# tangkk/audiomod

Hardware: NVIDIA B200
Metric: audio-sec/sec, 2048-pt PV pitch-shift, batched streams (higher is better)
Workload: dtype f32

## Files before the change

audiomod_b200/csrc/pv_engine.cu:

```cuda
#include <cuda_runtime.h>

#include <algorithm>
#include <chrono>
#include <cmath>
#include <cstdarg>
#include <cstdio>
#include <cstdlib>
#include <cstring>
#include <condition_variable>
#include <exception>
#include <functional>
#include <map>
#include <memory>
#include <mutex>
#include <new>
#include <string>
#include <thread>
#include <vector>

#include "../../include/pvgpu.h"
#include "pv_internal.h"
#include "pv_kernels.cuh"
#include "pv_plan.h"

#ifndef M_PI
#define M_PI 3.14159265358979323846
#endif

namespace pvgpu {

static thread_local std::string g_err;
const std::string &last_error_string() { return g_err; }
int fail(int code, const char *fmt, ...) {
    char buf[512];
    va_list ap;
    va_start(ap, fmt);
    vsnprintf(buf, sizeof buf, fmt, ap);
    va_end(ap);
    g_err = buf;
    return code;
}
template <class F> static int guarded(F f) {
    try {
        return f();
    } catch (const std::bad_alloc &) {
        return fail(PVGPU_ENOMEM, "out of host memory");
    } catch (const std::exception &e) {
        return fail(PVGPU_ESTATE, "unexpected failure: %s", e.what());
    }
}
#define CU(call)                                                                                      \
    do {                                                                                              \
        cudaError_t e_ = (call);                                                                      \
        if (e_ != cudaSuccess) return fail(e_ == cudaErrorMemoryAllocation ? PVGPU_ENOMEM : PVGPU_ECUDA, \
                                           "%s: %s (%s:%d)", #call, cudaGetErrorString(e_), __FILE__, __LINE__); \
    } while (0)

struct DevBuf {
    void *p = nullptr;
    size_t bytes = 0;
    ~DevBuf() { release(); }
    void release() { if (p) cudaFree(p); p = nullptr; bytes = 0; }
    cudaError_t ensure(size_t n) {
        if (n <= bytes) return cudaSuccess;
        release();
        cudaError_t e = cudaMalloc(&p, n);
        if (e == cudaSuccess) bytes = n;
        return e;
    }
    template <typename T> T *as() const { return (T *)p; }
};

struct PinnedArena {
    char *base = nullptr;
    size_t cap = 0, used = 0;
    ~PinnedArena() { if (base) cudaFreeHost(base); }
    void reserve(size_t bytes) {
        used = 0;
        if (bytes <= cap) return;
        if (base) cudaFreeHost(base);
        base = nullptr; cap = 0;
        const size_t want = bytes + bytes / 2 + 4096;
        if (cudaHostAlloc((void **)&base, want, cudaHostAllocDefault) == cudaSuccess) cap = want;
        else { cudaGetLastError(); base = nullptr; }
    }
    void *take(size_t bytes) {
        bytes = (bytes + 63) & ~(size_t)63;
        if (!base || used + bytes > cap) return nullptr;
        void *p = base + used;
        used += bytes;
        return p;
    }
};

static Config to_config(const pvgpu_config &c) {
    Config k;
    k.sample_rate = c.sample_rate; k.channels = c.channels; k.time_ratio = c.time_ratio; k.pitch_semitones = c.pitch_semitones;
    k.mode = c.mode; k.coremode = c.coremode; k.fftsize = c.fftsize; k.hopsize = c.hopsize;
    return k;
}

static int validate(const pvgpu_config *cfg) {
    if (!cfg) return fail(PVGPU_EINVAL, "null config");
    if (cfg->channels < 1 || cfg->channels > 16) return fail(PVGPU_EINVAL, "channels must be 1..16");
    if (cfg->sample_rate < 1000) return fail(PVGPU_EINVAL, "sample_rate too small");
    if (cfg->fftsize < 16 || cfg->fftsize > 16384) return fail(PVGPU_EINVAL, "fftsize must be 16..16384");
    return PVGPU_OK;
}

static void fill_info(const Derived &d, pvgpu_info *info) {
    info->fftsize = d.N; info->hop = d.hop; info->bins = d.H;
    info->pitch_scale = d.pitch_scale; info->hs_ratio = d.hs;
    info->resampler_active = d.rs.active ? 1 : 0;
    info->resampler_filt_len = (int)d.rs.filt_len;
    info->resampler_num = d.rs.num; info->resampler_den = d.rs.den;
    info->outbuf_capacity = d.outbuf_cap;
}

struct Pipeline {
    Derived d;
    Tables t;
    DevPlan p{};
    int device = 0;
    DevBuf b_window, b_twf, b_twi, b_stwf, b_stwi, b_perm, b_omega, b_rstab, b_rsquad, b_warp, b_tw2f, b_tw2i, b_tw3f, b_tw3i;
    DevBuf b_recs, b_norm, b_whisper, b_carmag, b_carph;
    long recs_base = 0, recs_count = 0;
    int64_t norm_base = 0;
    int max_consumed = 1;
    int max_out = 1;
    int ola_run = 16;
    bool fused = false;
    int fused_pref = -1;
    bool ola_ws = false;
    PostChain post{};
    FusedArgs fa{};
    std::vector<SliceRec> h_recs;
    DevBuf b_runs, b_rsent, b_rsfrac, b_rssteps;
    long run_origin = 0;
    int table_run = 1;
    int64_t launches = 0;
    bool profile = false;
    struct Span { int kind; cudaEvent_t a, b; };
    std::vector<Span> spans;
    size_t spans_used = 0;
    double kind_ms[8] = {0};
    int64_t kind_n[8] = {0};

    ~Pipeline() { for (auto &sp : spans) { cudaEventDestroy(sp.a); cudaEventDestroy(sp.b); } }

    Span *span_begin(int kind, cudaStream_t st) {
        if (!profile) return nullptr;
        if (spans_used == spans.size()) {
            Span sp{kind, nullptr, nullptr};
            if (cudaEventCreate(&sp.a) != cudaSuccess || cudaEventCreate(&sp.b) != cudaSuccess) return nullptr;
            spans.push_back(sp);
        }
        Span *sp = &spans[spans_used++];
        sp->kind = kind;
        cudaEventRecord(sp->a, st);
        return sp;
    }
    static void span_end(Span *sp, cudaStream_t st) { if (sp) cudaEventRecord(sp->b, st); }
    void collect_spans() {
        for (size_t i = 0; i < spans_used; ++i) {
            float ms = 0.f;
            if (cudaEventElapsedTime(&ms, spans[i].a, spans[i].b) == cudaSuccess) { kind_ms[spans[i].kind] += ms; kind_n[spans[i].kind] += 1; }
        }
        spans_used = 0;
    }

    int init(const pvgpu_config &cfg) {
        int ndev = 0;
        if (cudaGetDeviceCount(&ndev) != cudaSuccess || ndev == 0) return fail(PVGPU_ECUDA, "no CUDA device: the phase vocoder has no CPU fallback");
        if (cfg.device < 0 || cfg.device >= ndev) return fail(PVGPU_EINVAL, "device %d out of range (%d devices)", cfg.device, ndev);
        device = cfg.device;
        CU(cudaSetDevice(device));
        d = derive(to_config(cfg));
        if (d.hop < 1 || d.hop > d.N) return fail(PVGPU_EINVAL, "derived hop %d invalid for fft size %d", d.hop, d.N);
        t = make_tables(d.N, d.hop);
        if ((int)t.radix.size() > kMaxStages) return fail(PVGPU_EINVAL, "fft size too large");
        if (d.cepstral && !(d.N == 512 || d.N == 1024 || d.N == 2048 || d.N == 4096 || d.N == 8192))
            return fail(PVGPU_EINVAL, "the cepstral modes need an FFT size of 512..8192 (got %d)", d.N);
        CU(configure_kernels());
        p.N = d.N; p.H = d.H; p.half = d.N / 2; p.nc = d.N / 2; p.hop = d.hop;
        p.Hp = (d.H + 3) & ~3;
        p.nstages = (int)t.radix.size();
        for (int i = 0; i < p.nstages; ++i) { p.radix[i] = t.radix[i]; p.span[i] = t.span[i]; }
        p.inv_n = 1.f / d.N;
        p.two_pi_hop = 2 * M_PI * (size_t)d.hop;
        p.freq_comp = d.freq_comp;
        p.fixed_gain = d.fixed_gain;
        p.rs_active = (d.rs.active && !d.vocoder) ? 1 : 0;
        p.rs_direct = d.rs.direct ? 1 : 0;
        p.rs_num = d.rs.num; p.rs_den = d.rs.den; p.rs_filt_len = d.rs.filt_len; p.rs_oversample = d.rs.oversample;
        p.rs_int_adv = d.rs.int_adv; p.rs_frac_adv = d.rs.frac_adv;
        p.rs_table_len = (int)d.rs.table.size();
        if (!(d.robotic || d.whisper || d.vocoder || d.constant_mode) && d.cfg.coremode != 2 &&
            !(d.cfg.coremode == 1 && lock_smem_bytes(p, d.cfg.channels, max_peaks()) <= (size_t)200 * 1024) &&
            smem_phase_core(p, d.cfg.channels, max_peaks()) + 64 > (size_t)200 * 1024)
            return fail(PVGPU_EINVAL, "%d channels at FFT size %d need more shared memory per stream than the device has (the phase core keeps every channel's phase state on chip)",
                        d.cfg.channels, d.N);
        int rc;
        if ((rc = upload(b_window, t.window.data(), sizeof(float) * t.window.size()))) return rc;
        if ((rc = upload(b_twf, t.tw_fwd.data(), sizeof(float) * t.tw_fwd.size()))) return rc;
        if ((rc = upload(b_twi, t.tw_inv.data(), sizeof(float) * t.tw_inv.size()))) return rc;
        if ((rc = upload(b_stwf, t.stw_fwd.data(), sizeof(float) * t.stw_fwd.size()))) return rc;
        if ((rc = upload(b_stwi, t.stw_inv.data(), sizeof(float) * t.stw_inv.size()))) return rc;
        if ((rc = upload(b_perm, t.perm.data(), sizeof(uint16_t) * t.perm.size()))) return rc;
        if ((rc = upload(b_omega, t.omega.data(), sizeof(float) * t.omega.size()))) return rc;
        if (p.rs_active && (rc = upload(b_rstab, d.rs.table.data(), sizeof(float) * d.rs.table.size()))) return rc;
        p.window = b_window.as<float>();
        p.tw_fwd = b_twf.as<float2>(); p.tw_inv = b_twi.as<float2>();
        p.tw2_fwd = p.tw2_inv = p.tw3_fwd = p.tw3_inv = nullptr;
        {
            const int nc = d.N / 2;
            if (nc == 256 || nc == 512 || nc == 1024 || nc == 2048 || nc == 4096) {
                const bool r2 = nc == 512 || nc == 2048;
                const int mid = r2 ? 8 : 16, last = mid * 16, T = nc / 16;
                auto pair_table = [&](const std::vector<float> &tw, int M) {
                    std::vector<float> out((size_t)2 * 15 * M);
                    const int Fa = nc / (4 * M), Fb = nc / (16 * M);
                    for (int k = 0; k < M; ++k) {
                        int idx[15] = {k * Fa, 2 * k * Fa, 3 * k * Fa};
                        for (int j1 = 0; j1 < 4; ++j1) { const int kk = k + j1 * M; idx[3 + 3 * j1] = kk * Fb; idx[4 + 3 * j1] = 2 * kk * Fb; idx[5 + 3 * j1] = 3 * kk * Fb; }
                        for (int e = 0; e < 15; ++e) { out[2 * ((size_t)e * M + k)] = tw[2 * idx[e]]; out[2 * ((size_t)e * M + k) + 1] = tw[2 * idx[e] + 1]; }
                    }
                    return out;
                };
                auto single_table = [&](const std::vector<float> &tw) {
                    std::vector<float> out((size_t)2 * 12 * T);
                    for (int t = 0; t < T; ++t)
                        for (int q = 0; q < 4; ++q)
                            for (int m = 1; m <= 3; ++m) {
                                const int idx = m * (t + T * q);
                                const size_t o = (size_t)(3 * q + m - 1) * T + t;
                                out[2 * o] = tw[2 * idx]; out[2 * o + 1] = tw[2 * idx + 1];
                            }
                    return out;
                };
                const std::vector<float> f2 = pair_table(t.tw_fwd, mid), i2 = pair_table(t.tw_inv, mid);
                if ((rc = upload(b_tw2f, f2.data(), sizeof(float) * f2.size()))) return rc;
                if ((rc = upload(b_tw2i, i2.data(), sizeof(float) * i2.size()))) return rc;
                p.tw2_fwd = b_tw2f.as<float2>(); p.tw2_inv = b_tw2i.as<float2>();
                if (nc / last == 16 || nc / last == 4) {
                    const std::vector<float> f3 = nc / last == 16 ? pair_table(t.tw_fwd, last) : single_table(t.tw_fwd);
                    const std::vector<float> i3 = nc / last == 16 ? pair_table(t.tw_inv, last) : single_table(t.tw_inv);
                    if ((rc = upload(b_tw3f, f3.data(), sizeof(float) * f3.size()))) return rc;
                    if ((rc = upload(b_tw3i, i3.data(), sizeof(float) * i3.size()))) return rc;
                    p.tw3_fwd = b_tw3f.as<float2>(); p.tw3_inv = b_tw3i.as<float2>();
                }
            }
        }
        p.stw_fwd = b_stwf.as<float2>(); p.stw_inv = b_stwi.as<float2>();
        p.perm = b_perm.as<uint16_t>();
        p.omega = b_omega.as<float>();
        p.rs_table = b_rstab.as<float>();
        if (p.rs_active && !d.rs.direct) {
            const std::vector<float> &tab = d.rs.table;
            const int n = (int)tab.size();
            std::vector<float> quads((size_t)4 * n);
            for (int e = 0; e < n; ++e) {
                quads[4 * e + 0] = e >= 2 ? tab[e - 2] : 0.f;
                quads[4 * e + 1] = e >= 1 ? tab[e - 1] : 0.f;
                quads[4 * e + 2] = tab[e];
                quads[4 * e + 3] = e + 1 < n ? tab[e + 1] : 0.f;
            }
            if ((rc = upload(b_rsquad, quads.data(), sizeof(float) * quads.size()))) return rc;
        }
        p.rs_quads = b_rsquad.as<float4>();
        p.warp_tab = nullptr;
        if (cartesian() && cartesian_lock() && d.freq_comp != 0.f) {
            const int half = d.N / 2;
            std::vector<float> tab((size_t)4 * (half + 1));
            for (int i = 0; i <= half; ++i) {
                float wr = d.fixed_gain, wi = 0.f;
                int src = i;
                if (d.freq_comp > 1.0f || i < half) {
                    src = (int)std::lrint((float)i * d.freq_comp);
                    if (src > half) { src = 0; wr = 0.f; wi = 0.f; }
                    else {
                        const float dw = (float)((2 * M_PI * (size_t)d.hop * (i - src)) / (double)d.N);
                        wr = (float)(d.fixed_gain * std::cos((double)dw)); wi = (float)(d.fixed_gain * std::sin((double)dw));
                    }
                }
                tab[4 * i] = wr; tab[4 * i + 1] = wi; std::memcpy(&tab[4 * i + 2], &src, sizeof src); tab[4 * i + 3] = 0.f;
            }
            if ((rc = upload(b_warp, tab.data(), sizeof(float) * tab.size()))) return rc;
            p.warp_tab = b_warp.as<float4>();
        }
        return PVGPU_OK;
    }

    PinnedArena *arena = nullptr;
    bool staged_all = true;
    int h2d(void *dst, const void *src, size_t bytes, cudaStream_t st) {
        if (!bytes) return PVGPU_OK;
        void *pin = arena ? arena->take(bytes) : nullptr;
        if (pin) { std::memcpy(pin, src, bytes); src = pin; } else staged_all = false;
        CU(cudaMemcpyAsync(dst, src, bytes, cudaMemcpyHostToDevice, st));
        return PVGPU_OK;
    }
    struct RunScratch {
        std::vector<ResampleRun> runs;
        std::vector<unsigned> ent, steps, run_steps, be[kMaxBuckets], e2;
        std::vector<float> frac, coef, bf[kMaxBuckets], f2;
    } rsx;

    static int upload(DevBuf &b, const void *src, size_t bytes) {
        CU(b.ensure(bytes ? bytes : 4));
        if (bytes) CU(cudaMemcpy(b.p, src, bytes, cudaMemcpyHostToDevice));
        return PVGPU_OK;
    }

    int max_peaks() const { return p.half / 3 + 2; }

    bool cartesian_lock() const {
        if (!(d.cfg.coremode == 1 && !(d.robotic || d.whisper || d.vocoder || d.constant_mode))) return false;
        return lock_smem_bytes(p, d.cfg.channels, max_peaks()) <= (size_t)200 * 1024;
    }
    bool cartesian() const {
        const bool templated = p.N == 512 || p.N == 1024 || p.N == 2048 || p.N == 4096 || p.N == 8192;
        return templated && (d.robotic || d.whisper || d.vocoder || d.constant_mode || cartesian_lock());
    }
    void apply_mode(DevRows &g) const {
        g.spec = cartesian() ? 1 : 0;
        g.synth_kind = d.vocoder ? 0 : d.robotic ? 1 : d.whisper ? 2 : d.constant_mode ? 3 : cartesian_lock() ? 4 : 0;
        g.whisper = (d.whisper && cartesian()) ? b_whisper.as<float>() : nullptr;
        if (!cartesian()) g.synth_kind = 0;
    }

    int upload_schedule(const Scheduler &s, cudaStream_t st) {
        const auto &recs = s.recs();
        const auto &norm = s.norm();
        CU(b_recs.ensure(sizeof(SliceRec) * std::max<size_t>(recs.size(), 1)));
        CU(b_norm.ensure(sizeof(float) * std::max<size_t>(norm.size(), 1)));
        int rc;
        if ((rc = h2d(b_recs.p, recs.data(), sizeof(SliceRec) * recs.size(), st))) return rc;
        if ((rc = h2d(b_norm.p, norm.data(), sizeof(float) * norm.size(), st))) return rc;
        recs_base = s.recs_base();
        recs_count = (long)recs.size();
        norm_base = s.norm_base();
        for (const SliceRec &r : recs) { max_consumed = std::max(max_consumed, std::max(r.consumed, r.shift_inc)); max_out = std::max(max_out, r.n_res); }
        h_recs = recs;
        return PVGPU_OK;
    }

    int build_resample_runs(long origin, long end, int run, cudaStream_t st) {
        run_origin = origin;
        table_run = run;
        if (!p.rs_active) return PVGPU_OK;
        const int L = (int)p.rs_filt_len, ov = (int)p.rs_oversample, nb = p.rs_direct ? 1 : ov;
        if (L > kResPad) return fail(PVGPU_EINVAL, "resampler filter of %d taps is not supported (max %d)", L, kResPad);
        std::vector<ResampleRun> &runs = rsx.runs;
        std::vector<unsigned> &ent = rsx.ent, &steps = rsx.steps, &run_steps = rsx.run_steps;
        std::vector<float> &frac = rsx.frac;
        std::vector<unsigned> (&be)[kMaxBuckets] = rsx.be;
        std::vector<float> (&bf)[kMaxBuckets] = rsx.bf;
        runs.clear(); ent.clear(); frac.clear(); steps.clear(); run_steps.clear();
        for (long ka = origin; ka < end; ka += run) {
            const long kb = std::min<long>(ka + run, end);
            const SliceRec &ra = h_recs[ka - recs_base];
            ResampleRun hdr{};
            hdr.u_lo = std::max<int64_t>(0, ra.res_off + ra.rs_last - L + 1);
            hdr.out_first = ra.out_off;
            hdr.ent_off = (int)ent.size();
            {
                const int64_t u_lo_raw = ra.res_off + ra.rs_last - L + 1;
                long kmin = ka;
                while (kmin > recs_base && kmin > 0 && h_recs[kmin - recs_base].res_off > u_lo_raw && ka - kmin < ola_max_table_slices() - run - 1) --kmin;
                const long jmin = h_recs[kmin - recs_base].jlo;
                hdr.back_slices = (int)(ka - kmin);
                hdr.back_frames = (int)(ka - jmin);
                hdr.ola_base = h_recs[jmin - recs_base].ola_off;
            }
            for (int q = 0; q < nb; ++q) { be[q].clear(); bf[q].clear(); }
            for (long k = ka; k < kb; ++k) {
                const SliceRec &r = h_recs[k - recs_base];
                if (r.flags & 1) continue;
                int last = r.rs_last;
                uint32_t fn = r.rs_frac;
                for (int i = 0; i < r.n_write; ++i) {
                    const int bucket = p.rs_direct ? 0 : (int)(fn * (uint32_t)ov / p.rs_den);
                    const int64_t rel = r.res_off + last - L + 1 - hdr.u_lo + kResPad;
                    const int64_t orel = r.out_off - hdr.out_first + i;
                    if (rel < 0 || rel > 65535 || orel > 65534) return fail(PVGPU_ESTATE, "resampler run does not fit its packed work list");
                    be[bucket].push_back(((unsigned)rel << 16) | (unsigned)orel);
                    float fv;
                    if (p.rs_direct) { std::memcpy(&fv, &fn, sizeof fv); }
                    else fv = ((float)((fn * (uint32_t)ov) % p.rs_den)) / p.rs_den;
                    bf[bucket].push_back(fv);
                    last += p.rs_int_adv;
                    fn += (uint32_t)p.rs_frac_adv;
                    if (fn >= p.rs_den) { fn -= p.rs_den; ++last; }
                }
            }
            int pos = 0;
            for (int q = 0; q < nb; ++q) {
                if (!p.rs_direct) {
                    std::vector<unsigned> &e = be[q];
                    std::vector<float> &f = bf[q];
                    constexpr int kWin = 2048;
                    static const int win_env = []() { const char *v = getenv("PVGPU_RS_WIN"); int w = v ? atoi(v) : kWin; return w < 32 ? 32 : (w > kWin ? kWin : (w / 32) * 32); }();
                    for (size_t b0 = 0; b0 < e.size(); b0 += win_env) {
                        const int n = (int)std::min<size_t>(win_env, e.size() - b0), nrow = (n + 31) / 32;
                        static thread_local int rows[kWin / 32][32], spill[kWin];
                        int cnt[kWin / 32] = {}, nspill = 0;
                        int seen[32] = {};
                        for (int i = 0; i < n; ++i) {
// ... 1560 lines not shown
```

audiomod_b200/csrc/pv_kernels.cuh:

```cuda
#pragma once
#include <cstdint>
#include <cuda_runtime.h>

#include "pv_plan.h"

namespace pvgpu {

constexpr int kMaxStages = 8;

struct DevPlan {
    int N, H, half, nc, hop, Hp;
    int nstages;
    int radix[kMaxStages], span[kMaxStages];
    const float *window;
    const float2 *tw_fwd, *tw_inv;
    const float2 *tw2_fwd, *tw2_inv, *tw3_fwd, *tw3_inv;
    const float2 *stw_fwd, *stw_inv;
    const uint16_t *perm;
    const float *omega;
    float inv_n;
    double two_pi_hop;
    float freq_comp, fixed_gain;
    const float4 *warp_tab;
    int rs_active, rs_direct;
    uint32_t rs_num, rs_den, rs_filt_len, rs_oversample;
    int rs_int_adv, rs_frac_adv;
    const float *rs_table;
    const float4 *rs_quads;
    int rs_table_len;
};

struct DevRows {
    int rows;
    int channels;
    const void *in;
    int fmt;
    int64_t in_stride, in_base;
    const int64_t *n_in;
    float *mag, *phase;
    int F;
    float *frames;
    int Fr;
    void *out;
    int64_t out_stride, out_base;
    const int64_t *n_out;
    float *prev_phase, *prev_out;
    int *peaks;
    int maxpk;
    int *started;
    int2 *lock_hdr;
    float4 *lock_rec;
    int rec_stride;
    unsigned short *lock_map;
    float2 *lock_csn;
    float *lock_tail;
    int *lock_kind;
    float *lock_rot;
    float *ola_tail;
    float *res_hist;
    int zero_mask;
    long aux_base;
    int spec;
    int synth_kind;
    const float *whisper;
};

void launch_analyse(const DevPlan &p, const DevRows &g, long k0, int nframes, cudaStream_t st);
void launch_phase_core(const DevPlan &p, const DevRows &g, int coremode, const SliceRec *recs, long recs_base, long k0, int nframes, cudaStream_t st);
void launch_lock_peaks(const DevPlan &p, const DevRows &g, const SliceRec *recs, long recs_base, long k0, int nframes, cudaStream_t st);
void launch_lock_chain(const DevPlan &p, const DevRows &g, int nframes, cudaStream_t st);
int lock_rec_stride(const DevPlan &p, int maxpk);
void launch_fixed_phase(const DevPlan &p, const DevRows &g, const float *table ,
                        long k0, int nframes, cudaStream_t st);
void launch_synthesise(const DevPlan &p, const DevRows &g, const float *car_mag, const float *car_phase ,
                       long k0, int nframes, cudaStream_t st);
constexpr int kMaxBuckets = 8;
constexpr int kResPerThread = 4;
constexpr int kResBlock = 32 * kResPerThread;
constexpr int kResPad = 1024;
struct ResampleRun {
    int64_t u_lo;
    int64_t out_first;
    int ent_off;
    int padded;
    int64_t ola_base;
    int back_slices;
    int back_frames;
    int rsv[5];
    int step_off;
    int n_steps;
    int pad[1];
};
static_assert(sizeof(ResampleRun) == 72, "ResampleRun layout");

int ola_run_limit(const DevPlan &p, int run, int max_consumed, int max_out);
int ola_max_table_slices();
int ola_max_table_frames();
size_t lock_smem_bytes(const DevPlan &p, int channels, int maxpk);
void launch_ola_resample(const DevPlan &p, const DevRows &g, const SliceRec *recs, const float *norm, int64_t norm_base, long recs_base,
                         long k0, int nframes, int run, int max_consumed, const ResampleRun *runs, const unsigned *rs_ent, const float *rs_frac,
                         const unsigned *rs_steps, long run_origin, cudaStream_t st);
bool launch_ola_resample_ws(const DevPlan &p, const DevRows &g, const SliceRec *recs, const float *norm, int64_t norm_base, long recs_base, long k0, int nframes,
                            int run, int max_consumed, const ResampleRun *runs, const unsigned *rs_ent, const float *rs_frac, const unsigned *rs_steps,
                            long run_origin, cudaStream_t st, cudaError_t *err);
struct FusedArgs {
    const SliceRec *recs; long recs_base;
    const float *norm; int64_t norm_base;
    long k0; int nf;
    int run;
    int acc_len;
    int in_len;
    int hist_len;
    int ws;
    const ResampleRun *runs; const unsigned *rs_ent; const float *rs_frac; const unsigned *rs_steps; long run_origin;
    const float *car_mag, *car_phase;
};
int fused_frames_in_flight(int N);
bool fused_plan(const DevPlan &p, int frames_per_chunk, int max_shift, int max_consumed, int max_out, size_t smem_limit, int force_run, bool want_ws, FusedArgs *out);
cudaError_t launch_synth_ola(const DevPlan &p, const DevRows &g, const FusedArgs &a, cudaStream_t st);

bool launch_cepstral(const DevPlan &p, const DevRows &g, float env_comp, int nframes, cudaStream_t st);
constexpr int kMaxPostFx = 12;
enum { kFxGain = 1, kFxCompressor = 2, kFxLimiter = 3, kFxBiquad = 4 };
struct PostFx { int kind; int delay; float p[6]; };
struct PostChain { int n; PostFx fx[kMaxPostFx]; };
int postchain_state_stride(const PostChain &pc);
void launch_postchain_reset(const PostChain &pc, float *state, int rows, cudaStream_t st);
void launch_postchain(const DevRows &g, const PostChain &pc, float *state, int64_t col0, int64_t col1, cudaStream_t st);

void launch_place_rows(float *dst, int64_t dst_pitch, const float *src, int64_t src_pitch, int width, int rows, cudaStream_t st);
void launch_ring_rows(float *dst, int64_t dst_pitch, int64_t dst_off, int64_t dst_mask, const float *src, int64_t src_pitch, int64_t src_off, int64_t src_mask,
                      int width, int rows, cudaStream_t st);

void launch_test_atan2f(int64_t n, const float *y, const float *x, float *out, cudaStream_t st);
void launch_test_princarg(int64_t n, const double *a, double *out, cudaStream_t st);

size_t smem_analyse(const DevPlan &p);
size_t smem_phase_core(const DevPlan &p, int channels, int maxpk);
size_t smem_synthesise(const DevPlan &p);

cudaError_t configure_kernels();

}
```

audiomod_b200/csrc/pv_lock.cuh:

```cuda
#pragma once

constexpr int kLockRun = 32;

__device__ __forceinline__ bool lock_is_peak(float qb, float qmax) {
    if (!(qb > qmax)) return false;
    if (qb > __fmul_rn(qmax, 1.00000048f) && qb > 1e-30f) return true;
    return __fsqrt_rn(qb) > __fsqrt_rn(qmax);
}

__host__ __device__ inline int lock_peaks_map_offset(int half, int C, int maxpk) { return (3 * half + 8 + 2 * C * half + 3 * maxpk + 1 + 32 + 3) & ~3; }
inline size_t lock_peaks_smem(int half, int C, int maxpk) {
    return sizeof(float) * (size_t)lock_peaks_map_offset(half, C, maxpk) + sizeof(unsigned short) * (size_t)C * half + 4 * sizeof(float) * (size_t)C * maxpk;
}
inline size_t lock_chain_smem(int half, int C, int maxpk) { return sizeof(float) * ((size_t)C * 2 * maxpk + (size_t)C * half) + sizeof(int) * 2 * (size_t)C; }

template <int N> struct LockShape {
    static constexpr int kHalf = N / 2;
    static constexpr int E = N == 8192 ? 8 : 4;
    static constexpr int kThreads = kHalf / E;
    static constexpr int kMinBlocks = 1024 / kThreads > 16 ? 16 : 1024 / kThreads;
    static constexpr int kMaxPk = kHalf / 3 + 2;
};

template <int N, int kC>
__global__ void __launch_bounds__(LockShape<N>::kThreads, LockShape<N>::kMinBlocks) k_lock_peaks(const DevPlan p, const DevRows g, const SliceRec *__restrict__ recs,
                                                                                                   long recs_base, long k0, int nframes) {
    constexpr int E = LockShape<N>::E;
    extern __shared__ float smem[];
    constexpr int half = LockShape<N>::kHalf, maxpk = LockShape<N>::kMaxPk, nthr = LockShape<N>::kThreads, nwarp = nthr / 32;
    const int C = kC ? kC : g.channels;
    float *s_q = smem;
    float *s_cre = s_q + half + 8;
    float *s_cim = s_cre + half;
    float *s_A = s_cim + half;
    float *s_B = s_A + C * half;
    int *s_pk0 = (int *)(s_B + C * half);
    int *s_pk1 = s_pk0 + maxpk;
    int *s_start = s_pk1 + maxpk;
    int *s_wsum = s_start + maxpk + 1;
    unsigned short *s_map = (unsigned short *)(smem + lock_peaks_map_offset(half, C, maxpk));
    const int stream = blockIdx.y, tid = threadIdx.x;
    const int lane = tid & 31, warp = tid >> 5;
    const int b0 = tid * E;
    const int fa = blockIdx.x * kLockRun, fb = min(fa + kLockRun, nframes);
    const int f_first = (k0 + fa > 0) ? fa - 1 : fa;
    float *s_cph = (float *)(s_map + C * half);
    int *s_cpk = (int *)(s_cph + C * 2 * maxpk);
    unsigned cache_ok = 0, cache_side = 0;

    float pre[E], pim[E];
    int ff = f_first, cf = 0;
    const int64_t row0 = (int64_t)stream * C;
    const int64_t ch_step = (int64_t)g.F * p.Hp;
    const int64_t fr_step = (int64_t)p.Hp - (C - 1) * ch_step;
    const float *fre = g.mag + (row0 * g.F + max(f_first, 0)) * p.Hp + b0;
    const float *fim = g.phase + (row0 * g.F + max(f_first, 0)) * p.Hp + b0;
    auto fetch = [&]() {
        const float *sr, *si;
        if (ff < 0) {
            sr = g.lock_tail + (row0 + cf) * 2 * p.Hp + b0;
            si = sr + p.Hp;
        } else {
            sr = fre; si = fim;
            const int64_t step = (kC == 1 || cf == C - 1) ? fr_step : ch_step;
            fre += step; fim += step;
        }
        if (kC == 1 || ++cf == C) { cf = 0; ++ff; }
#pragma unroll
        for (int e = 0; e < E; e += 4) {
            const float4 r4 = *(const float4 *)(sr + e);
            const float4 i4 = *(const float4 *)(si + e);
            pre[e] = r4.x; pre[e + 1] = r4.y; pre[e + 2] = r4.z; pre[e + 3] = r4.w;
            pim[e] = i4.x; pim[e + 1] = i4.y; pim[e + 2] = i4.z; pim[e + 3] = i4.w;
        }
    };
    if (f_first < fb) fetch();
    if (tid < 4) { s_q[tid] = 0.f; s_q[half + 4 + tid] = 0.f; }
    int *s_prev = s_pk0, *s_cur = s_pk1;
    int nprev = 0;
    const float hopf = (float)p.hop;
    const SliceRec *__restrict__ rec_f = recs + (k0 - recs_base);

    for (int f = f_first; f < fb; ++f) {
        const bool warm = f < fa;
        const bool k_is_0 = k0 + f == 0;
        for (int c = 0; c < C; ++c) {
            float *A = s_A + c * half, *B = s_B + c * half;
            unsigned short *map_c = s_map + c * half;
            const unsigned short *map_p = s_map + (c == 0 ? C - 1 : c - 1) * half;
            float re[E], im[E], q[E];
#pragma unroll
            for (int e = 0; e < E; ++e) {
                re[e] = pre[e]; im[e] = pim[e];
                q[e] = __fadd_rn(__fmul_rn(re[e], re[e]), __fmul_rn(im[e], im[e]));
            }
#pragma unroll
            for (int e = 0; e < E; e += 4) {
                *(float4 *)(s_q + 4 + b0 + e) = make_float4(q[e], q[e + 1], q[e + 2], q[e + 3]);
                *(float4 *)(s_cre + b0 + e) = make_float4(re[e], re[e + 1], re[e + 2], re[e + 3]);
                *(float4 *)(s_cim + b0 + e) = make_float4(im[e], im[e + 1], im[e + 2], im[e + 3]);
            }
            __syncthreads();
            float w[E + 4];
            w[0] = s_q[4 + b0 - 2]; w[1] = s_q[4 + b0 - 1];
#pragma unroll
            for (int e = 0; e < E; ++e) w[2 + e] = q[e];
            w[E + 2] = s_q[4 + b0 + E]; w[E + 3] = s_q[4 + b0 + E + 1];
            unsigned flags = 0, unsure = 0;
#pragma unroll
            for (int e = 0; e < E; ++e) {
                const float qmax = fmaxf(fmaxf(w[e], w[e + 1]), fmaxf(w[e + 3], w[e + 4]));
                const bool cand = w[e + 2] > qmax;
                const bool sure = w[e + 2] > fmaxf(__fmul_rn(qmax, 1.00000048f), 1e-30f);
                flags |= (unsigned)sure << e;
                unsure |= (unsigned)(cand && !sure) << e;
            }
            while (unsure) {
                const int e = __ffs(unsure) - 1;
                unsure &= unsure - 1;
                const float qmax = fmaxf(fmaxf(s_q[4 + b0 + e - 2], s_q[4 + b0 + e - 1]), fmaxf(s_q[4 + b0 + e + 1], s_q[4 + b0 + e + 2]));
                flags |= (unsigned)lock_is_peak(s_q[4 + b0 + e], qmax) << e;
            }
            if (tid == 0) flags &= ~3u;
            if (tid == nthr - 1) flags &= ~(3u << (E - 2));
            const int cnt = __popc(flags);
            const unsigned lt = (1u << lane) - 1;
            const unsigned b1 = __ballot_sync(0xffffffffu, cnt >= 1), b2 = __ballot_sync(0xffffffffu, cnt >= 2);
            int excl = __popc(b1 & lt) + __popc(b2 & lt), wtot = __popc(b1) + __popc(b2);
            if (E == 8) { const unsigned b3 = __ballot_sync(0xffffffffu, cnt >= 3); excl += __popc(b3 & lt); wtot += __popc(b3); }
            const int incl = excl + cnt;
            if (lane == 31) s_wsum[warp] = wtot;
            if (ff < fb) fetch();
            __syncthreads();
            int ws = lane < nwarp ? s_wsum[lane] : 0;
#pragma unroll
            for (int d = 1; d < nwarp; d <<= 1) {
                const int v = __shfl_up_sync(0xffffffffu, ws, d);
                if (lane >= d) ws += v;
            }
            const int npk = __shfl_sync(0xffffffffu, ws, nwarp - 1);
            int base = __shfl_sync(0xffffffffu, ws, (warp + 31) & 31);
            base = (warp == 0 ? 0 : base) + incl - cnt;
            if (flags) {
                s_cur[base] = b0 + __ffs(flags) - 1;
                if (cnt > 1) s_cur[base + cnt - 1] = b0 + 31 - __clz(flags);
                if (E == 8 && cnt > 2) s_cur[base + 1] = b0 + __ffs(flags & (flags - 1)) - 1;
            }
            const int64_t slot = (row0 + c) * g.F + f;
            const bool first = k_is_0 && c == 0;
            const int kind = first ? 0 : (npk == 0 || nprev == 0) ? 1 : 2;
            const bool lock_now = !warm && kind == 2;
            __syncthreads();
            for (int r = tid; r <= npk; r += nthr)
                s_start[r] = r == 0 ? 0 : r == npk ? half : (s_cur[r - 1] + s_cur[r] + 1) >> 1;
            if (lock_now) {
                const float phase_inc = (float)rec_f[f].phase_inc;
                float4 *__restrict__ out = g.lock_rec + slot * g.rec_stride;
                const bool cached = (cache_ok >> c) & 1;
                const int cs = (cache_side >> c) & 1;
                const float *cph = s_cph + (c * 2 + cs) * maxpk;
                const int *cpk = s_cpk + (c * 2 + cs) * maxpk;
                float *nph = s_cph + (c * 2 + (cs ^ 1)) * maxpk;
                int *npb = s_cpk + (c * 2 + (cs ^ 1)) * maxpk;
                for (int r = tid; r < npk; r += nthr) {
                    const int p2 = s_cur[r];
                    const int r1 = map_p[p2];
                    const int q1 = s_prev[r1];
                    const int j = (r1 > 0 && q1 - p2 == p2 - s_prev[r1 - 1]) ? r1 - 1 : r1;
                    const int p1 = s_prev[j];
                    const int ridx = map_c[p1];
                    const float php = pv_atan2f_fast(s_cim[p2], s_cre[p2]);
                    float a;
                    if (k_is_0) a = 0.f;
                    else if (cached && cpk[ridx] == p1) a = cph[ridx];
                    else a = pv_atan2f_fast(B[p1], A[p1]);
                    const float avg_p = (float)((double)(p1 + p2) * 0.5);
                    const float pomega = (float)__dmul_rn(__dmul_rn(p.two_pi_hop, (double)__fsub_rn(avg_p, 1.0f)), (double)p.inv_n);
                    const float dphi = (float)__dadd_rn((double)pomega, princarg_fast((double)sub3_rn(php, a, pomega)));
                    const float adv = __fdiv_rn(__fmul_rn(dphi, phase_inc), hopf);
                    out[r] = make_float4(php, a, adv, __int_as_float(p1 | (ridx << 16)));
                    nph[r] = php; npb[r] = p2;
                }
            } else if (!warm && kind == 1) {
                const float phase_inc = (float)rec_f[f].phase_inc;
                float *__restrict__ adv_o = (float *)(g.lock_rec + slot * g.rec_stride);
                float *__restrict__ a_o = adv_o + half;
                unsigned short *__restrict__ ridx_o = g.lock_map + slot * half;
#pragma unroll 1
                for (int e = 0; e < E; ++e) {
                    const int i = b0 + e;
                    const float omega = __ldg(&p.omega[i]);
                    const float phi = pv_atan2f_fast(s_cim[i], s_cre[i]);
                    const float a = k_is_0 ? 0.f : pv_atan2f_fast(B[i], A[i]);
                    const float dphi = (float)__dadd_rn((double)omega, princarg_fast((double)sub3_rn(phi, a, omega)));
                    adv_o[i] = __fdiv_rn(__fmul_rn(dphi, phase_inc), hopf);
                    a_o[i] = a;
                    ridx_o[i] = map_c[i];
                }
            }
            __syncthreads();
            if (npk > 0) {
                unsigned short rg[E];
#pragma unroll
                for (int e = 0; e < E; ++e) {
                    const int lo = base - 1 + __popc(flags & ((2u << e) - 1));
                    rg[e] = (unsigned short)(lo + (b0 + e >= s_start[lo + 1]));
                }
#pragma unroll
                for (int e = 0; e < E; e += 4) {
                    const uint2 v = make_uint2(rg[e] | ((unsigned)rg[e + 1] << 16), rg[e + 2] | ((unsigned)rg[e + 3] << 16));
                    *(uint2 *)(map_c + b0 + e) = v;
                    if (lock_now) *(uint2 *)(g.lock_map + slot * half + b0 + e) = v;
                }
            }
#pragma unroll
            for (int e = 0; e < E; e += 4) {
                *(float4 *)(A + b0 + e) = make_float4(re[e], re[e + 1], re[e + 2], re[e + 3]);
                *(float4 *)(B + b0 + e) = make_float4(im[e], im[e + 1], im[e + 2], im[e + 3]);
            }
            if (lock_now) { cache_ok |= 1u << c; cache_side ^= 1u << c; }
            else cache_ok &= ~(1u << c);
            if (!warm && tid == 0) g.lock_hdr[slot] = make_int2(npk, kind);
            { int *tsw = s_prev; s_prev = s_cur; s_cur = tsw; }
            nprev = npk;
        }
    }
}

__device__ __noinline__ void lock_chain_classic(int half, const float *__restrict__ adv_i, const unsigned short *__restrict__ ridx_i, float *__restrict__ gre,
                                                float *__restrict__ gim, int kp, const float *rot_p, float *out_c) {
    const float *__restrict__ a_i = adv_i + half;
    for (int i = threadIdx.x; i < half; i += blockDim.x) {
        const float a = a_i[i];
        float po;
        if (kp == 2) po = (float)princarg_fast((double)__fadd_rn(a, rot_p[ridx_i[i]]));
        else if (kp == 1) po = out_c[i];
        else if (kp == 3) po = a;
        else po = 0.f;
        const float outp = (float)princarg_fast((double)__fadd_rn(po, adv_i[i]));
        out_c[i] = outp;
        const float re = gre[i], im = gim[i];
        const float m = __fsqrt_rn(__fadd_rn(__fmul_rn(re, re), __fmul_rn(im, im)));
        float sn, cs;
        sincosf(outp, &sn, &cs);
        gre[i] = m * cs; gim[i] = m * sn;
    }
}

constexpr int kChainThreads = 128;
template <int kC>
__global__ void __launch_bounds__(kChainThreads, 10) k_lock_chain(const DevPlan p, const DevRows g, int nframes) {
    extern __shared__ float smem[];
    const int half = p.half, C = kC ? kC : g.channels, maxpk = g.maxpk;
    float *s_rot = smem;
    float *s_out = s_rot + C * 2 * maxpk;
    int *s_kind = (int *)(s_out + C * half);
    int *s_flip = s_kind + C;
    const int stream = blockIdx.x, tid = threadIdx.x;
    constexpr int nthr = kChainThreads;
    const int64_t row0 = (int64_t)stream * C;
    for (int c = 0; c < C; ++c) {
        const int64_t row = row0 + c;
        const int kd = g.lock_kind[row];
        if (kd == 2) for (int i = tid; i < maxpk; i += nthr) s_rot[c * 2 * maxpk + i] = g.lock_rot[row * maxpk + i];
        if (kd == 1) for (int i = tid; i < half; i += nthr) s_out[c * half + i] = g.prev_out[row * half + i];
        if (tid == 0) { s_kind[c] = kd; s_flip[c] = 0; }
    }
    __syncthreads();
    int kind_r[kC ? kC : 1], flip_r[kC ? kC : 1];
#pragma unroll
    for (int c = 0; c < kC; ++c) { kind_r[c] = s_kind[c]; flip_r[c] = 0; }
    const int rs = g.rec_stride;
    const int64_t ch_step = g.F, fr_step = 1 - (int64_t)(C - 1) * g.F;
    const int2 *__restrict__ hdr_f = g.lock_hdr + row0 * g.F;
    const float4 *__restrict__ rec_f = g.lock_rec + row0 * g.F * rs + tid;
    const float4 *__restrict__ rec_c = rec_f;
    float2 *__restrict__ csn_c = g.lock_csn + row0 * g.F * maxpk;
    int2 hdr_n = make_int2(0, 0);
    float4 rec_n0 = make_float4(0.f, 0.f, 0.f, 0.f), rec_n1 = rec_n0;
    int cf = 0, left = nframes * C;
    auto fetch = [&]() {
        hdr_n = *hdr_f;
        rec_n0 = rec_f[0];
        rec_n1 = rec_f[nthr];
        const int64_t step = (kC == 1 || cf == C - 1) ? fr_step : ch_step;
        if (kC != 1) cf = cf == C - 1 ? 0 : cf + 1;
        hdr_f += step; rec_f += step * rs;
        --left;
    };
    if (left > 0) fetch();
    for (int f = 0; f < nframes; ++f) {
#pragma unroll
        for (int c = 0; c < C; ++c) {
            const int2 hdr = hdr_n;
            const float4 rec0 = rec_n0, rec1 = rec_n1;
            if (left > 0) fetch();
            int kp, fl;
            if (kC) { kp = kind_r[c]; fl = flip_r[c]; }
            else { kp = s_kind[c]; fl = s_flip[c]; __syncthreads(); }
            const float *rot_p = s_rot + (c * 2 + fl) * maxpk;
            float *rot_n = s_rot + (c * 2 + (fl ^ 1)) * maxpk;
            float *out_c = s_out + c * half;
            int new_kind;
            if (hdr.y == 2) {
                const int npk = hdr.x;
                for (int r = tid; r < npk; r += nthr) {
                    const float4 rec = r == tid ? rec0 : r == tid + nthr ? rec1 : rec_c[r - tid];
                    const float php = rec.x, a = rec.y, adv = rec.z;
                    const int link = __float_as_int(rec.w);
                    float po;
                    if (kp == 2) po = (float)princarg_fast((double)__fadd_rn(a, rot_p[link >> 16]));
                    else if (kp == 1) po = out_c[link & 0xffff];
                    else if (kp == 3) po = a;
                    else po = 0.f;
                    const float target = (float)princarg_fast((double)__fadd_rn(po, adv));
                    const float rot = (float)princarg_fast((double)__fsub_rn(target, php));
                    rot_n[r] = rot;
                    float sn, cs;
                    sincosf(rot, &sn, &cs);
                    csn_c[r] = make_float2(cs, sn);
                }
                new_kind = 2;
            } else if (hdr.y == 0) {
                new_kind = 3;
            } else {
                const int64_t slot = (row0 + c) * g.F + f;
                lock_chain_classic(half, (const float *)(g.lock_rec + slot * rs), g.lock_map + slot * half, g.mag + slot * p.Hp, g.phase + slot * p.Hp, kp, rot_p, out_c);
                new_kind = 1;
            }
            if (kC) { kind_r[c] = new_kind; if (new_kind == 2) flip_r[c] = fl ^ 1; }
            else if (tid == 0) { s_kind[c] = new_kind; if (new_kind == 2) s_flip[c] = fl ^ 1; }
            const int64_t step = (kC == 1 || c == C - 1) ? fr_step : ch_step;
            rec_c += step * rs; csn_c += step * maxpk;
            __syncthreads();
        }
    }
    if (kC && tid == 0) {
#pragma unroll
        for (int c = 0; c < kC; ++c) { s_kind[c] = kind_r[c]; s_flip[c] = flip_r[c]; }
    }
    __syncthreads();
    for (int c = 0; c < C; ++c) {
        const int64_t row = row0 + c;
        const int kd = s_kind[c];
        if (kd == 2) for (int i = tid; i < maxpk; i += nthr) g.lock_rot[row * maxpk + i] = s_rot[(c * 2 + s_flip[c]) * maxpk + i];
        if (kd == 1) for (int i = tid; i < half; i += nthr) g.prev_out[row * half + i] = s_out[c * half + i];
        if (tid == 0) g.lock_kind[row] = kd;
    }
}
```

Baseline: 196,800.

## Restructure lock-peaks kernel to cut barriers and shared-memory traffic

```diff
diff --git a/audiomod_b200/csrc/pv_engine.cu b/audiomod_b200/csrc/pv_engine.cu
--- a/audiomod_b200/csrc/pv_engine.cu
+++ b/audiomod_b200/csrc/pv_engine.cu
@@ -122,7 +122,7 @@
     Tables t;
     DevPlan p{};
     int device = 0;
-    DevBuf b_window, b_twf, b_twi, b_stwf, b_stwi, b_perm, b_omega, b_rstab, b_rsquad, b_warp, b_tw2f, b_tw2i, b_tw3f, b_tw3i;
+    DevBuf b_window, b_twf, b_twi, b_stwf, b_stwi, b_perm, b_omega, b_pomega, b_rstab, b_rsquad, b_warp, b_tw2f, b_tw2i, b_tw3f, b_tw3i;
     DevBuf b_recs, b_norm, b_whisper, b_carmag, b_carph;
     long recs_base = 0, recs_count = 0;
     int64_t norm_base = 0;
@@ -208,6 +208,14 @@
         if ((rc = upload(b_stwi, t.stw_inv.data(), sizeof(float) * t.stw_inv.size()))) return rc;
         if ((rc = upload(b_perm, t.perm.data(), sizeof(uint16_t) * t.perm.size()))) return rc;
         if ((rc = upload(b_omega, t.omega.data(), sizeof(float) * t.omega.size()))) return rc;
+        {
+            std::vector<float> pom((size_t)2 * p.half);
+            for (int s = 0; s < 2 * p.half; ++s) {
+                const float avg_p = (float)((double)s * 0.5);
+                pom[s] = (float)((p.two_pi_hop * (double)(avg_p - 1.0f)) * (double)p.inv_n);
+            }
+            if ((rc = upload(b_pomega, pom.data(), sizeof(float) * pom.size()))) return rc;
+        }
         if (p.rs_active && (rc = upload(b_rstab, d.rs.table.data(), sizeof(float) * d.rs.table.size()))) return rc;
         p.window = b_window.as<float>();
         p.tw_fwd = b_twf.as<float2>(); p.tw_inv = b_twi.as<float2>();
@@ -254,6 +262,7 @@
         p.stw_fwd = b_stwf.as<float2>(); p.stw_inv = b_stwi.as<float2>();
         p.perm = b_perm.as<uint16_t>();
         p.omega = b_omega.as<float>();
+        p.pomega = b_pomega.as<float>();
         p.rs_table = b_rstab.as<float>();
         if (p.rs_active && !d.rs.direct) {
             const std::vector<float> &tab = d.rs.table;
diff --git a/audiomod_b200/csrc/pv_kernels.cuh b/audiomod_b200/csrc/pv_kernels.cuh
--- a/audiomod_b200/csrc/pv_kernels.cuh
+++ b/audiomod_b200/csrc/pv_kernels.cuh
@@ -18,6 +18,7 @@
     const float2 *stw_fwd, *stw_inv;
     const uint16_t *perm;
     const float *omega;
+    const float *pomega;
     float inv_n;
     double two_pi_hop;
     float freq_comp, fixed_gain;
diff --git a/audiomod_b200/csrc/pv_lock.cuh b/audiomod_b200/csrc/pv_lock.cuh
--- a/audiomod_b200/csrc/pv_lock.cuh
+++ b/audiomod_b200/csrc/pv_lock.cuh
@@ -1,6 +1,6 @@
 #pragma once
 
-constexpr int kLockRun = 32;
+constexpr int kLockRun = 64;
 
 __device__ __forceinline__ bool lock_is_peak(float qb, float qmax) {
     if (!(qb > qmax)) return false;
@@ -8,9 +8,9 @@
     return __fsqrt_rn(qb) > __fsqrt_rn(qmax);
 }
 
-__host__ __device__ inline int lock_peaks_map_offset(int half, int C, int maxpk) { return (3 * half + 8 + 2 * C * half + 3 * maxpk + 1 + 32 + 3) & ~3; }
+__host__ __device__ inline int lock_peaks_map_offset(int half, int C, int maxpk) { return (2 * (C + 1) * half + 2 * (maxpk + 1) + 32 + 3) & ~3; }
 inline size_t lock_peaks_smem(int half, int C, int maxpk) {
-    return sizeof(float) * (size_t)lock_peaks_map_offset(half, C, maxpk) + sizeof(unsigned short) * (size_t)C * half + 4 * sizeof(float) * (size_t)C * maxpk;
+    return sizeof(float) * (size_t)lock_peaks_map_offset(half, C, maxpk) + sizeof(unsigned short) * (size_t)(C + 1) * half + 4 * sizeof(float) * (size_t)C * maxpk;
 }
 inline size_t lock_chain_smem(int half, int C, int maxpk) { return sizeof(float) * ((size_t)C * 2 * maxpk + (size_t)C * half) + sizeof(int) * 2 * (size_t)C; }
 
@@ -22,6 +22,8 @@
     static constexpr int kMaxPk = kHalf / 3 + 2;
 };
 
+constexpr int kLockPkLo = -(1 << 20), kLockPkHi = 1 << 20;
+
 template <int N, int kC>
 __global__ void __launch_bounds__(LockShape<N>::kThreads, LockShape<N>::kMinBlocks) k_lock_peaks(const DevPlan p, const DevRows g, const SliceRec *__restrict__ recs,
                                                                                                    long recs_base, long k0, int nframes) {
@@ -29,26 +31,23 @@
     extern __shared__ float smem[];
     constexpr int half = LockShape<N>::kHalf, maxpk = LockShape<N>::kMaxPk, nthr = LockShape<N>::kThreads, nwarp = nthr / 32;
     const int C = kC ? kC : g.channels;
-    float *s_q = smem;
-    float *s_cre = s_q + half + 8;
-    float *s_cim = s_cre + half;
-    float *s_A = s_cim + half;
-    float *s_B = s_A + C * half;
-    int *s_pk0 = (int *)(s_B + C * half);
-    int *s_pk1 = s_pk0 + maxpk;
-    int *s_start = s_pk1 + maxpk;
-    int *s_wsum = s_start + maxpk + 1;
+    float *s_spec = smem;
+    int *s_pk0 = (int *)(s_spec + (C + 1) * 2 * half) + 1;
+    int *s_pk1 = s_pk0 + maxpk + 1;
+    int *s_wsum = s_pk1 + maxpk;
     unsigned short *s_map = (unsigned short *)(smem + lock_peaks_map_offset(half, C, maxpk));
+    float *s_cph = (float *)(s_map + (C + 1) * half);
+    int *s_cpk = (int *)(s_cph + C * 2 * maxpk);
+    unsigned cache_ok = 0, cache_side = 0;
     const int stream = blockIdx.y, tid = threadIdx.x;
     const int lane = tid & 31, warp = tid >> 5;
     const int b0 = tid * E;
     const int fa = blockIdx.x * kLockRun, fb = min(fa + kLockRun, nframes);
     const int f_first = (k0 + fa > 0) ? fa - 1 : fa;
-    float *s_cph = (float *)(s_map + C * half);
-    int *s_cpk = (int *)(s_cph + C * 2 * maxpk);
-    unsigned cache_ok = 0, cache_side = 0;
 
     float pre[E], pim[E];
+    float2 pere = make_float2(0.f, 0.f), peim = pere;
+    const int edge_off = (lane == 0 && tid > 0) ? -2 : (lane == 31 && tid < nthr - 1) ? E : 0;
     int ff = f_first, cf = 0;
     const int64_t row0 = (int64_t)stream * C;
     const int64_t ch_step = (int64_t)g.F * p.Hp;
@@ -73,11 +72,13 @@
             pre[e] = r4.x; pre[e + 1] = r4.y; pre[e + 2] = r4.z; pre[e + 3] = r4.w;
             pim[e] = i4.x; pim[e + 1] = i4.y; pim[e + 2] = i4.z; pim[e + 3] = i4.w;
         }
+        if (edge_off) { pere = *(const float2 *)(sr + edge_off); peim = *(const float2 *)(si + edge_off); }
     };
     if (f_first < fb) fetch();
-    if (tid < 4) { s_q[tid] = 0.f; s_q[half + 4 + tid] = 0.f; }
+    if (tid == 0) { s_pk0[-1] = kLockPkLo; s_pk1[-1] = kLockPkLo; }
     int *s_prev = s_pk0, *s_cur = s_pk1;
     int nprev = 0;
+    int slot = 0;
     const float hopf = (float)p.hop;
     const SliceRec *__restrict__ rec_f = recs + (k0 - recs_base);
 
@@ -85,27 +86,29 @@
         const bool warm = f < fa;
         const bool k_is_0 = k0 + f == 0;
         for (int c = 0; c < C; ++c) {
-            float *A = s_A + c * half, *B = s_B + c * half;
-            unsigned short *map_c = s_map + c * half;
-            const unsigned short *map_p = s_map + (c == 0 ? C - 1 : c - 1) * half;
+            const int slot_c = slot == C ? 0 : slot + 1, slot_p = slot == 0 ? C : slot - 1;
+            float *cre = s_spec + slot * 2 * half, *cim = cre + half;
+            const float *A = s_spec + slot_c * 2 * half, *B = A + half;
+            unsigned short *map_n = s_map + slot * half;
+            const unsigned short *map_c = s_map + slot_c * half;
+            const unsigned short *map_p = s_map + slot_p * half;
             float re[E], im[E], q[E];
 #pragma unroll
             for (int e = 0; e < E; ++e) {
                 re[e] = pre[e]; im[e] = pim[e];
                 q[e] = __fadd_rn(__fmul_rn(re[e], re[e]), __fmul_rn(im[e], im[e]));
             }
-#pragma unroll
-            for (int e = 0; e < E; e += 4) {
-                *(float4 *)(s_q + 4 + b0 + e) = make_float4(q[e], q[e + 1], q[e + 2], q[e + 3]);
-                *(float4 *)(s_cre + b0 + e) = make_float4(re[e], re[e + 1], re[e + 2], re[e + 3]);
-                *(float4 *)(s_cim + b0 + e) = make_float4(im[e], im[e + 1], im[e + 2], im[e + 3]);
-            }
-            __syncthreads();
             float w[E + 4];
-            w[0] = s_q[4 + b0 - 2]; w[1] = s_q[4 + b0 - 1];
 #pragma unroll
             for (int e = 0; e < E; ++e) w[2 + e] = q[e];
-            w[E + 2] = s_q[4 + b0 + E]; w[E + 3] = s_q[4 + b0 + E + 1];
+            {
+                const float eq0 = __fadd_rn(__fmul_rn(pere.x, pere.x), __fmul_rn(peim.x, peim.x));
+                const float eq1 = __fadd_rn(__fmul_rn(pere.y, pere.y), __fmul_rn(peim.y, peim.y));
+                const float l0 = __shfl_up_sync(0xffffffffu, q[E - 2], 1), l1 = __shfl_up_sync(0xffffffffu, q[E - 1], 1);
+                const float r0 = __shfl_down_sync(0xffffffffu, q[0], 1), r1 = __shfl_down_sync(0xffffffffu, q[1], 1);
+                w[0] = lane == 0 ? eq0 : l0; w[1] = lane == 0 ? eq1 : l1;
+                w[E + 2] = lane == 31 ? eq0 : r0; w[E + 3] = lane == 31 ? eq1 : r1;
+            }
             unsigned flags = 0, unsure = 0;
 #pragma unroll
             for (int e = 0; e < E; ++e) {
@@ -115,11 +118,11 @@
                 flags |= (unsigned)sure << e;
                 unsure |= (unsigned)(cand && !sure) << e;
             }
-            while (unsure) {
-                const int e = __ffs(unsure) - 1;
-                unsure &= unsure - 1;
-                const float qmax = fmaxf(fmaxf(s_q[4 + b0 + e - 2], s_q[4 + b0 + e - 1]), fmaxf(s_q[4 + b0 + e + 1], s_q[4 + b0 + e + 2]));
-                flags |= (unsigned)lock_is_peak(s_q[4 + b0 + e], qmax) << e;
+            if (unsure) {
+#pragma unroll
+                for (int e = 0; e < E; ++e)
+                    if ((unsure >> e) & 1)
+                        flags |= (unsigned)lock_is_peak(w[e + 2], fmaxf(fmaxf(w[e], w[e + 1]), fmaxf(w[e + 3], w[e + 4]))) << e;
             }
             if (tid == 0) flags &= ~3u;
             if (tid == nthr - 1) flags &= ~(3u << (E - 2));
@@ -128,10 +131,14 @@
             const unsigned b1 = __ballot_sync(0xffffffffu, cnt >= 1), b2 = __ballot_sync(0xffffffffu, cnt >= 2);
             int excl = __popc(b1 & lt) + __popc(b2 & lt), wtot = __popc(b1) + __popc(b2);
             if (E == 8) { const unsigned b3 = __ballot_sync(0xffffffffu, cnt >= 3); excl += __popc(b3 & lt); wtot += __popc(b3); }
-            const int incl = excl + cnt;
             if (lane == 31) s_wsum[warp] = wtot;
+            __syncthreads();
+#pragma unroll
+            for (int e = 0; e < E; e += 4) {
+                *(float4 *)(cre + b0 + e) = make_float4(re[e], re[e + 1], re[e + 2], re[e + 3]);
+                *(float4 *)(cim + b0 + e) = make_float4(im[e], im[e + 1], im[e + 2], im[e + 3]);
+            }
             if (ff < fb) fetch();
-            __syncthreads();
             int ws = lane < nwarp ? s_wsum[lane] : 0;
 #pragma unroll
             for (int d = 1; d < nwarp; d <<= 1) {
@@ -140,22 +147,35 @@
             }
             const int npk = __shfl_sync(0xffffffffu, ws, nwarp - 1);
             int base = __shfl_sync(0xffffffffu, ws, (warp + 31) & 31);
-            base = (warp == 0 ? 0 : base) + incl - cnt;
+            base = (warp == 0 ? 0 : base) + excl;
             if (flags) {
                 s_cur[base] = b0 + __ffs(flags) - 1;
                 if (cnt > 1) s_cur[base + cnt - 1] = b0 + 31 - __clz(flags);
                 if (E == 8 && cnt > 2) s_cur[base + 1] = b0 + __ffs(flags & (flags - 1)) - 1;
             }
-            const int64_t slot = (row0 + c) * g.F + f;
+            if (tid == 0) s_cur[npk] = kLockPkHi;
+            const int64_t slot_g = (row0 + c) * g.F + f;
             const bool first = k_is_0 && c == 0;
             const int kind = first ? 0 : (npk == 0 || nprev == 0) ? 1 : 2;
             const bool lock_now = !warm && kind == 2;
             __syncthreads();
-            for (int r = tid; r <= npk; r += nthr)
-                s_start[r] = r == 0 ? 0 : r == npk ? half : (s_cur[r - 1] + s_cur[r] + 1) >> 1;
+            if (npk > 0) {
+                unsigned short rg[E];
+#pragma unroll
+                for (int e = 0; e < E; ++e) {
+                    const int lo = base - 1 + __popc(flags & ((2u << e) - 1));
+                    rg[e] = (unsigned short)(lo + (b0 + e >= ((s_cur[lo] + s_cur[lo + 1] + 1) >> 1)));
+                }
+#pragma unroll
+                for (int e = 0; e < E; e += 4) {
+                    const uint2 v = make_uint2(rg[e] | ((unsigned)rg[e + 1] << 16), rg[e + 2] | ((unsigned)rg[e + 3] << 16));
+                    *(uint2 *)(map_n + b0 + e) = v;
+                    if (lock_now) *(uint2 *)(g.lock_map + slot_g * half + b0 + e) = v;
+                }
+            }
             if (lock_now) {
                 const float phase_inc = (float)rec_f[f].phase_inc;
-                float4 *__restrict__ out = g.lock_rec + slot * g.rec_stride;
+                float4 *__restrict__ out = g.lock_rec + slot_g * g.rec_stride;
                 const bool cached = (cache_ok >> c) & 1;
                 const int cs = (cache_side >> c) & 1;
                 const float *cph = s_cph + (c * 2 + cs) * maxpk;
@@ -169,13 +189,12 @@
                     const int j = (r1 > 0 && q1 - p2 == p2 - s_prev[r1 - 1]) ? r1 - 1 : r1;
                     const int p1 = s_prev[j];
                     const int ridx = map_c[p1];
-                    const float php = pv_atan2f_fast(s_cim[p2], s_cre[p2]);
+                    const float pomega = __ldg(&p.pomega[p1 + p2]);
+                    const float php = pv_atan2f_fast(cim[p2], cre[p2]);
                     float a;
                     if (k_is_0) a = 0.f;
                     else if (cached && cpk[ridx] == p1) a = cph[ridx];
                     else a = pv_atan2f_fast(B[p1], A[p1]);
-                    const float avg_p = (float)((double)(p1 + p2) * 0.5);
-                    const float pomega = (float)__dmul_rn(__dmul_rn(p.two_pi_hop, (double)__fsub_rn(avg_p, 1.0f)), (double)p.inv_n);
                     const float dphi = (float)__dadd_rn((double)pomega, princarg_fast((double)sub3_rn(php, a, pomega)));
                     const float adv = __fdiv_rn(__fmul_rn(dphi, phase_inc), hopf);
                     out[r] = make_float4(php, a, adv, __int_as_float(p1 | (ridx << 16)));
@@ -183,14 +202,14 @@
                 }
             } else if (!warm && kind == 1) {
                 const float phase_inc = (float)rec_f[f].phase_inc;
-                float *__restrict__ adv_o = (float *)(g.lock_rec + slot * g.rec_stride);
+                float *__restrict__ adv_o = (float *)(g.lock_rec + slot_g * g.rec_stride);
                 float *__restrict__ a_o = adv_o + half;
-                unsigned short *__restrict__ ridx_o = g.lock_map + slot * half;
+                unsigned short *__restrict__ ridx_o = g.lock_map + slot_g * half;
 #pragma unroll 1
                 for (int e = 0; e < E; ++e) {
                     const int i = b0 + e;
                     const float omega = __ldg(&p.omega[i]);
-                    const float phi = pv_atan2f_fast(s_cim[i], s_cre[i]);
+                    const float phi = pv_atan2f_fast(cim[i], cre[i]);
                     const float a = k_is_0 ? 0.f : pv_atan2f_fast(B[i], A[i]);
                     const float dphi = (float)__dadd_rn((double)omega, princarg_fast((double)sub3_rn(phi, a, omega)));
                     adv_o[i] = __fdiv_rn(__fmul_rn(dphi, phase_inc), hopf);
@@ -198,31 +217,12 @@
                     ridx_o[i] = map_c[i];
                 }
             }
-            __syncthreads();
-            if (npk > 0) {
-                unsigned short rg[E];
-#pragma unroll
-                for (int e = 0; e < E; ++e) {
-                    const int lo = base - 1 + __popc(flags & ((2u << e) - 1));
-                    rg[e] = (unsigned short)(lo + (b0 + e >= s_start[lo + 1]));
-                }
-#pragma unroll
-                for (int e = 0; e < E; e += 4) {
-                    const uint2 v = make_uint2(rg[e] | ((unsigned)rg[e + 1] << 16), rg[e + 2] | ((unsigned)rg[e + 3] << 16));
-                    *(uint2 *)(map_c + b0 + e) = v;
-                    if (lock_now) *(uint2 *)(g.lock_map + slot * half + b0 + e) = v;
-                }
-            }
-#pragma unroll
-            for (int e = 0; e < E; e += 4) {
-                *(float4 *)(A + b0 + e) = make_float4(re[e], re[e + 1], re[e + 2], re[e + 3]);
-                *(float4 *)(B + b0 + e) = make_float4(im[e], im[e + 1], im[e + 2], im[e + 3]);
-            }
             if (lock_now) { cache_ok |= 1u << c; cache_side ^= 1u << c; }
             else cache_ok &= ~(1u << c);
-            if (!warm && tid == 0) g.lock_hdr[slot] = make_int2(npk, kind);
+            if (!warm && tid == 0) g.lock_hdr[slot_g] = make_int2(npk, kind);
             { int *tsw = s_prev; s_prev = s_cur; s_cur = tsw; }
             nprev = npk;
+            slot = slot_c;
         }
     }
 }
```

Result: faster. 199,800 (median of 6 runs) (+1.5%).
